# sec-bit/ckb-zkp

Measured on AMD Instinct MI355X. Metric: Groth16 proofs/sec (2^20 constraints, BN256), higher is better.
Workload: dtype u32 limbs (256-bit Montgomery integers); 1 GPU; Groth16 prove, MiMC-chain R1CS, 1048570 constraints (domain 2^20), 1258284 aux, bn254, G1 x4 + G2 x1 MSM + 4 NTT (7 in the reference: evaluation-form key); curve=bn254, log_domain=20, parallelism=independent proofs x1

## Files before the change

### ckb_zkp_amd/csrc/capi.hip

```cpp
#include <cstdint>
#include <cstdlib>
#include <cstring>

#include "ctx.hpp"
#include "host_field.hpp"
#include "internal.hpp"
#include "ipa.hpp"

using namespace zkp;

namespace {

template <class Fn>
int32_t guarded(zkp_ctx* ctx, Fn&& fn) {
  if (!ctx) return ZKP_ERR_BAD_ARG;
  std::lock_guard<std::recursive_mutex> lk(ctx->mu);
  try {
    ZKP_HIP(hipSetDevice(ctx->device));
    fn();
    return ZKP_OK;
  } catch (const StatusError& e) {
    return e.status;
  } catch (const HipError& e) {
    ctx->last_error = std::string(e.what) + ": " + hipGetErrorString(e.e);
    fprintf(stderr, "[zkp_accel] HIP error %s at line %d: %s\n", hipGetErrorString(e.e), e.line, e.what);
    return e.e == hipErrorOutOfMemory ? ZKP_ERR_OOM : ZKP_ERR_DEVICE;
  } catch (const std::bad_alloc&) {
    return ZKP_ERR_OOM;
  } catch (...) {
    return ZKP_ERR_DEVICE;
  }
}

template <class Fn>
int32_t guarded_multi(zkp_ctx* root, Fn&& fn) {
  if (!root) return ZKP_ERR_BAD_ARG;
  std::vector<std::unique_lock<std::recursive_mutex>> member_locks;
  std::unique_lock<std::recursive_mutex> root_lock(root->mu);
  for (size_t k = 1; k < root->devs.size(); k++) member_locks.emplace_back(root->devs[k]->mu);
  return guarded(root, fn);
}

zkp_cfg cfg_from_env() {
  zkp_cfg c;
  auto num = [](const char* name, long long dflt) { const char* e = getenv(name); return e ? atoll(e) : dflt; };
  auto off = [](const char* name) { const char* e = getenv(name); return e && atoi(e) == 0; };
  c.lanes = (int)num("ZKP_LANES", 0);
  c.msm_batch_lanes = (int)std::max<long long>(1, std::min<long long>(num("ZKP_BATCH_LANES", 1), zkp_ctx::N_LANES));
  c.msm_c = (int)num("ZKP_MSM_C", 0);
  c.msm_c_g2 = (int)num("ZKP_MSM_C_G2", 0);
  if (const char* e = getenv("ZKP_MSM_CHUNK")) c.msm_chunk = (long long)strtoull(e, nullptr, 0);
  if (const char* e = getenv("ZKP_TABLE_BUDGET_GB")) c.table_budget_gb = atof(e);
  c.h_lagrange = !off("ZKP_H_LAGRANGE");
  c.c_fold = !off("ZKP_C_FOLD");
  c.host_affine = !off("ZKP_HOST_AFFINE");
  c.lfold_heavy_cost = num("ZKP_LFOLD_HEAVY_COST", c.lfold_heavy_cost);
  if (const char* e = getenv("ZKP_MULTI_EXCHANGE")) c.multi_exchange = !strcmp(e, "rccl") ? ZKP_EXCHANGE_RCCL : !strcmp(e, "peer") ? ZKP_EXCHANGE_PEER : ZKP_EXCHANGE_AUTO;
  c.multi_exchange_timeout_ms = (int)num("ZKP_MULTI_EXCHANGE_TIMEOUT_MS", c.multi_exchange_timeout_ms);
  c.multi_wm_split = (int)num("ZKP_MULTI_WM_SPLIT", -1);
  return c;
}

int32_t apply_config(zkp_cfg* c, const zkp_ctx_config* u) {
  if (!u) return ZKP_OK;
  if (u->struct_size < sizeof(uint32_t) * 2) return ZKP_ERR_BAD_ARG;
  zkp_ctx_config f{};
  memcpy(&f, u, std::min<size_t>(u->struct_size, sizeof f));
  auto tri_ok = [](int32_t v) { return v == ZKP_DEFAULT || v == ZKP_ON || v == ZKP_OFF; };
  if (f.lanes < 0 || f.lanes > zkp_ctx::N_LANES || f.msm_batch_lanes < 0 || f.msm_batch_lanes > zkp_ctx::N_LANES) return ZKP_ERR_BAD_ARG;
  for (int32_t b : {f.msm_window_bits, f.msm_window_bits_g2})
    if (b != 0 && (b < 2 || b > 22)) return ZKP_ERR_BAD_ARG;
  if (f.msm_chunk_points < -1 || (f.msm_chunk_points > 0 && f.msm_chunk_points < 1024)) return ZKP_ERR_BAD_ARG;
  if (!(f.table_budget_gb >= 0.0) || f.c_fold_heavy_cost < 0 || f.multi_exchange_timeout_ms < 0) return ZKP_ERR_BAD_ARG;
  if (!tri_ok(f.h_evaluation_form) || !tri_ok(f.c_fold) || !tri_ok(f.host_affine) || !tri_ok(f.multi_witness_split)) return ZKP_ERR_BAD_ARG;
  if (f.multi_exchange < ZKP_EXCHANGE_AUTO || f.multi_exchange > ZKP_EXCHANGE_PEER) return ZKP_ERR_BAD_ARG;
  if (f.lanes) c->lanes = f.lanes;
  if (f.msm_batch_lanes) c->msm_batch_lanes = f.msm_batch_lanes;
  if (f.msm_window_bits) c->msm_c = f.msm_window_bits;
  if (f.msm_window_bits_g2) c->msm_c_g2 = f.msm_window_bits_g2;
  if (f.msm_chunk_points) c->msm_chunk = f.msm_chunk_points < 0 ? 0 : f.msm_chunk_points;
  if (f.table_budget_gb > 0.0) c->table_budget_gb = f.table_budget_gb;
  if (f.h_evaluation_form) c->h_lagrange = f.h_evaluation_form == ZKP_ON;
  if (f.c_fold) c->c_fold = f.c_fold == ZKP_ON;
  if (f.host_affine) c->host_affine = f.host_affine == ZKP_ON;
  if (f.c_fold_heavy_cost) c->lfold_heavy_cost = f.c_fold_heavy_cost;
  if (f.multi_exchange) c->multi_exchange = f.multi_exchange;
  if (f.multi_exchange_timeout_ms) c->multi_exchange_timeout_ms = f.multi_exchange_timeout_ms;
  if (f.multi_witness_split) c->multi_wm_split = f.multi_witness_split == ZKP_ON ? 1 : 0;
  return ZKP_OK;
}

}

extern "C" {

const char* zkp_status_string(int32_t s) {
  switch (s) {
    case ZKP_OK: return "ok";
    case ZKP_ERR_BAD_ARG: return "bad argument";
    case ZKP_ERR_UNSUPPORTED_CURVE: return "unsupported curve";
    case ZKP_ERR_DOMAIN_TOO_LARGE: return "domain too large (PolynomialDegreeTooLarge)";
    case ZKP_ERR_OOM: return "out of device memory";
    case ZKP_ERR_DEVICE: return "HIP device error / no gfx950 device (there is no CPU fallback)";
    case ZKP_ERR_BAD_HANDLE: return "bad handle";
    case ZKP_ERR_INVALID_POINT: return "malformed point / not on the curve / not in the prime-order subgroup (InvalidData)";
    default: return "unknown status";
  }
}

const char* zkp_version(void) { return "zkp_accel 0.7.1 (gfx950)"; }

int32_t zkp_ctx_get_config(zkp_ctx* ctx, zkp_ctx_config* out) {
  if (!ctx || !out) return ZKP_ERR_BAD_ARG;
  return guarded(ctx, [&] {
    const zkp_cfg& c = ctx->cfg;
    zkp_ctx_config f{};
    f.struct_size = sizeof f;
    f.lanes = c.lanes;
    f.msm_batch_lanes = c.msm_batch_lanes;
    f.msm_window_bits = c.msm_c;
    f.msm_window_bits_g2 = c.msm_c_g2;
    f.msm_chunk_points = c.msm_chunk > 0 ? c.msm_chunk : -1;
    f.table_budget_gb = c.table_budget_gb;
    f.h_evaluation_form = c.h_lagrange ? ZKP_ON : ZKP_OFF;
    f.c_fold = c.c_fold ? ZKP_ON : ZKP_OFF;
    f.host_affine = c.host_affine ? ZKP_ON : ZKP_OFF;
    f.c_fold_heavy_cost = c.lfold_heavy_cost;
    f.multi_exchange = c.multi_exchange;
    f.multi_exchange_timeout_ms = c.multi_exchange_timeout_ms;
    f.multi_witness_split = c.multi_wm_split < 0 ? ZKP_DEFAULT : c.multi_wm_split ? ZKP_ON : ZKP_OFF;
    *out = f;
  });
}

int32_t zkp_ctx_create(zkp_ctx** out, int device_id) { return zkp_ctx_create_ex(out, device_id, nullptr); }

int32_t zkp_ctx_create_ex(zkp_ctx** out, int device_id, const zkp_ctx_config* user_cfg) {
  if (!out) return ZKP_ERR_BAD_ARG;
  *out = nullptr;
  zkp_cfg cfg = cfg_from_env();
  if (int32_t st = apply_config(&cfg, user_cfg); st != ZKP_OK) return st;
  int count = 0;
  if (hipGetDeviceCount(&count) != hipSuccess || count <= 0 || device_id < 0 || device_id >= count) {
    fprintf(stderr, "[zkp_accel] no usable HIP device (count=%d, requested %d); there is no CPU fallback\n", count,
            device_id);
    return ZKP_ERR_DEVICE;
  }
  zkp_ctx* ctx = new (std::nothrow) zkp_ctx();
  if (!ctx) return ZKP_ERR_OOM;
  ctx->device = device_id;
  ctx->cfg = cfg;
  int32_t st = guarded(ctx, [&] {
    ZKP_HIP(hipEventCreate(&ctx->ev0));
    ZKP_HIP(hipEventCreate(&ctx->ev1));
    ZKP_HIP(hipEventCreate(&ctx->ev2));
    ZKP_HIP(hipEventCreate(&ctx->ev3));
    for (int l = 0; l < zkp_ctx::N_LANES; l++) {
      zkp_lane& L = ctx->lanes[l];
      ZKP_HIP(hipStreamCreateWithFlags(&L.stream, hipStreamNonBlocking));
      ZKP_HIP(hipEventCreateWithFlags(&L.ev_fork, hipEventDisableTiming));
      ZKP_HIP(hipEventCreateWithFlags(&L.ev_a, hipEventDisableTiming));
      ZKP_HIP(hipEventCreateWithFlags(&L.ev_b1, hipEventDisableTiming));
      ZKP_HIP(hipHostMalloc(reinterpret_cast<void**>(&L.host_proof), 1100));
      for (int i = 0; i < zkp_lane::N_WS; i++) {
        ZKP_HIP(hipEventCreateWithFlags(&L.ws[i].done, hipEventDisableTiming));
        ZKP_HIP(hipEventCreateWithFlags(&L.ws[i].sorted, hipEventDisableTiming));
        ZKP_HIP(hipEventCreateWithFlags(&L.ws[i].l1_done, hipEventDisableTiming));
        ZKP_HIP(hipEventCreateWithFlags(&L.ws[i].acc_done, hipEventDisableTiming));
        if (i > 0) {
          ZKP_HIP(hipStreamCreateWithFlags(&L.ws[i].stream, hipStreamNonBlocking));
          L.ws[i].own_stream = true;
        }
      }
    }
  });
  if (st != ZKP_OK) {
    (void)zkp_ctx_destroy(ctx);
    return st;
  }
  *out = ctx;
  return ZKP_OK;
}

int32_t zkp_ctx_create_multi(zkp_ctx** out, const int* device_ids, int n_devices) {
  return zkp_ctx_create_multi_ex(out, device_ids, n_devices, nullptr);
}

int32_t zkp_ctx_create_multi_ex(zkp_ctx** out, const int* device_ids, int n_devices, const zkp_ctx_config* cfg) {
  if (!out || !device_ids || n_devices < 1 || n_devices > 64) return ZKP_ERR_BAD_ARG;
  *out = nullptr;
  zkp_ctx* root = nullptr;
  int32_t st = zkp_ctx_create_ex(&root, device_ids[0], cfg);
  if (st != ZKP_OK) return st;
  root->devs.push_back(root);
  for (int k = 1; k < n_devices; k++) {
    zkp_ctx* m = nullptr;
    st = zkp_ctx_create_ex(&m, device_ids[k], cfg);
    if (st != ZKP_OK) {
      (void)zkp_ctx_destroy(root);
      return st;
    }
    root->devs.push_back(m);
  }
  for (int a = 0; a < n_devices; a++)
    for (int b = 0; b < n_devices; b++) {
      if (device_ids[a] == device_ids[b]) continue;
      int can = 0;
      if (hipDeviceCanAccessPeer(&can, device_ids[a], device_ids[b]) == hipSuccess && can) {
        (void)hipSetDevice(device_ids[a]);
        hipError_t e = hipDeviceEnablePeerAccess(device_ids[b], 0);
        if (e != hipSuccess) (void)hipGetLastError();
      }
    }
  (void)hipSetDevice(device_ids[0]);
  *out = root;
  return ZKP_OK;
}
int32_t zkp_ctx_num_devices(zkp_ctx* ctx, int32_t* n) {
  if (!ctx || !n) return ZKP_ERR_BAD_ARG;
  *n = ctx->devs.empty() ? 1 : (int32_t)ctx->devs.size();
  return ZKP_OK;
}
int32_t zkp_ctx_device(zkp_ctx* ctx, int32_t rank, zkp_ctx** member) {
  if (!ctx || !member) return ZKP_ERR_BAD_ARG;
  if (ctx->devs.empty()) {
    if (rank != 0) return ZKP_ERR_BAD_ARG;
    *member = ctx;
    return ZKP_OK;
  }
  if (rank < 0 || rank >= (int32_t)ctx->devs.size()) return ZKP_ERR_BAD_ARG;
  *member = ctx->devs[rank];
  return ZKP_OK;
}

int32_t zkp_ctx_destroy(zkp_ctx* ctx) {
  if (!ctx) return ZKP_ERR_BAD_ARG;
  { std::lock_guard<std::recursive_mutex> wait_for_calls_in_flight(ctx->mu); }
  for (size_t k = 1; k < ctx->devs.size(); k++) (void)zkp_ctx_destroy(ctx->devs[k]);
  ctx->devs.clear();
  (void)hipSetDevice(ctx->device);
  (void)hipDeviceSynchronize();
  ntt_free_tables(ctx);
  msm_free_all(ctx);
  for (hipEvent_t e : {ctx->ev0, ctx->ev1, ctx->ev2, ctx->ev3})
    if (e) (void)hipEventDestroy(e);
  for (int l = 0; l < zkp_ctx::N_LANES; l++) {
    zkp_lane& L = ctx->lanes[l];
    for (hipEvent_t e : {L.ev_fork, L.ev_a, L.ev_b1})
      if (e) (void)hipEventDestroy(e);
    if (L.host_proof) (void)hipHostFree(L.host_proof);
    for (int i = 0; i < zkp_lane::N_WS; i++) {
      if (L.ws[i].done) (void)hipEventDestroy(L.ws[i].done);
      if (L.ws[i].sorted) (void)hipEventDestroy(L.ws[i].sorted);
      if (L.ws[i].l1_done) (void)hipEventDestroy(L.ws[i].l1_done);
      if (L.ws[i].acc_done) (void)hipEventDestroy(L.ws[i].acc_done);
      if (L.ws[i].own_stream && L.ws[i].stream) (void)hipStreamDestroy(L.ws[i].stream);
    }
    if (L.own_stream && L.stream) (void)hipStreamDestroy(L.stream);
  }
  if (ctx->pinned) (void)hipHostFree(ctx->pinned);
  delete ctx;
  return ZKP_OK;
}

int32_t zkp_ctx_set_stream(zkp_ctx* ctx, void* s) {
  return guarded(ctx, [&] {
    zkp_lane& L = ctx->lanes[0];
    ZKP_HIP(hipStreamSynchronize(L.stream));
    if (s) {
      if (L.own_stream && L.stream) (void)hipStreamDestroy(L.stream);
      L.stream = reinterpret_cast<hipStream_t>(s);
      L.own_stream = false;
    } else if (!L.own_stream) {
      ZKP_HIP(hipStreamCreateWithFlags(&L.stream, hipStreamNonBlocking));
      L.own_stream = true;
    }
  });
}

int32_t zkp_ctx_sync(zkp_ctx* ctx) {
  return guarded(ctx, [&] { ZKP_HIP(hipStreamSynchronize(ctx->cur->stream)); });
}

int32_t zkp_dev_alloc(zkp_ctx* ctx, size_t bytes, void** dptr) {
  if (!dptr) return ZKP_ERR_BAD_ARG;
  return guarded(ctx, [&] {
    *dptr = nullptr;
    if (hipMalloc(dptr, bytes ? bytes : 16) != hipSuccess) throw StatusError{ZKP_ERR_OOM};
  });
}
int32_t zkp_dev_free(zkp_ctx* ctx, void* dptr) {
  return guarded(ctx, [&] {
    ZKP_HIP(hipStreamSynchronize(ctx->cur->stream));
    if (dptr) ZKP_HIP(hipFree(dptr));
  });
}
int32_t zkp_h2d(zkp_ctx* ctx, void* dst, const void* src, size_t bytes) {
  if (bytes && (!dst || !src)) return ZKP_ERR_BAD_ARG;
  return guarded(ctx, [&] {
    if (bytes) ZKP_HIP(hipMemcpyAsync(dst, src, bytes, hipMemcpyHostToDevice, ctx->cur->stream));
    ZKP_HIP(hipStreamSynchronize(ctx->cur->stream));
  });
}
int32_t zkp_d2h(zkp_ctx* ctx, void* dst, const void* src, size_t bytes) {
  if (bytes && (!dst || !src)) return ZKP_ERR_BAD_ARG;
  return guarded(ctx, [&] {
    if (bytes) ZKP_HIP(hipMemcpyAsync(dst, src, bytes, hipMemcpyDeviceToHost, ctx->cur->stream));
    ZKP_HIP(hipStreamSynchronize(ctx->cur->stream));
  });
}
int32_t zkp_timer_start(zkp_ctx* ctx) {
  return guarded(ctx, [&] { ZKP_HIP(hipEventRecord(ctx->ev0, ctx->cur->stream)); });
// ... 423 lines not shown
```

### ckb_zkp_amd/csrc/ctx.hpp

```cpp
#pragma once
#include <hip/hip_runtime.h>
#include <stdint.h>

#include <map>
#include <mutex>
#include <memory>
#include <string>
#include <unordered_map>
#include <vector>

#include "../../include/zkp_accel.h"

namespace zkp {

struct HipError {
  hipError_t e;
  const char* what;
  int line;
};

#define ZKP_HIP(call)                                                   \
  do {                                                                  \
    hipError_t _e = (call);                                             \
    if (_e != hipSuccess) throw ::zkp::HipError{_e, #call, __LINE__};   \
// ... 32 lines not shown
  DevBuf& operator=(const DevBuf&) = delete;
};

struct NttTables {
  int log_n = 0, h = 0;
  uint32_t* w_lo = nullptr;
  uint32_t* w_hi = nullptr;
  uint32_t* wi_lo = nullptr;
  uint32_t* wi_hi = nullptr;
  uint32_t* g_lo = nullptr;
  uint32_t* g_hi = nullptr;
  uint32_t* gi_lo = nullptr;
  uint32_t* gi_hi = nullptr;
  uint32_t* sub_fwd = nullptr;
  uint32_t* sub_inv = nullptr;
  uint32_t* n_inv = nullptr;
  void* block = nullptr;
  uint32_t* full_fwd[8] = {};
  uint32_t* full_inv[8] = {};
  uint32_t* full_g = nullptr;
  uint32_t* full_gi = nullptr;
  uint32_t* g_hi_n = nullptr;
  uint32_t* full_g_n = nullptr;
  std::vector<void*> extra;
};

struct BasesEntry;

struct MsmWorkspace {
  hipStream_t stream = nullptr;
  bool own_stream = false;
  hipEvent_t done = nullptr;
  hipEvent_t sorted = nullptr;
  hipEvent_t l1_done = nullptr;
  uint32_t chain_nb = 0;
  size_t chain_xb = 0;
  hipEvent_t acc_done = nullptr;
  DevBuf keys, vals, keys2, vals2, sort_tmp, offsets, buckets, tmp, out, sched, scan_tmp, scan_tmp2, partial, redo;
};
struct Groth16Timing {
  zkp_groth16_timing t{};
};

}

struct zkp_lane {
  hipStream_t stream = nullptr;
  bool own_stream = true;
  static constexpr int N_WS = 4;
  static constexpr int N_WS_MSM = N_WS;
  zkp::MsmWorkspace ws[N_WS];
  zkp::DevBuf ntt_scratch;
  hipEvent_t ev_fork = nullptr, ev_a = nullptr, ev_b1 = nullptr;
  uint32_t* host_proof = nullptr;
  bool host_tail = false;
  bool busy = false;
};

struct zkp_cfg {
  int lanes = 0;
  int msm_batch_lanes = 1;
  int msm_c = 0, msm_c_g2 = 0;
  long long msm_chunk = (long long)3 << 19;
  double table_budget_gb = 0;
  bool h_lagrange = true, c_fold = true, host_affine = true;
  long long lfold_heavy_cost = 0;
  int multi_exchange = 0;
  int multi_exchange_timeout_ms = 30000;
  int multi_wm_split = -1;
};

struct zkp_ctx {
  int device = 0;
  zkp_cfg cfg;
  std::recursive_mutex mu;
  static constexpr int N_LANES = 8;
  static constexpr int N_WS = zkp_lane::N_WS;
  zkp_lane lanes[N_LANES];
  zkp_lane* cur = &lanes[0];
  int cur_idx = 0;
  hipEvent_t ev0 = nullptr, ev1 = nullptr;
  hipEvent_t ev2 = nullptr, ev3 = nullptr;
  bool profiling = false;
  size_t table_bytes = 0;
  bool msm_defer_reduce = false;
  int msm_acc_into = -1;
  int msm_bucket_ws = -1;
  bool dbg_skip_k8 = false;
  bool batch_mode = false;
  std::map<std::pair<int, int>, zkp::NttTables> ntt_tables;
  zkp::DevBuf ntt_io, poly_tmp, poly_consts, spmv_list;
  zkp::DevBuf msm_scalars, msm_misc, var_bases;
  uint32_t* pinned = nullptr;
  size_t pinned_cap = 0;
  std::unordered_map<uint64_t, std::shared_ptr<zkp::BasesEntry>> bases;
  uint64_t next_handle = 1;
  zkp_groth16_timing last_timing{};
  zkp_marlin_timing last_marlin_timing{};
  std::string last_error;
  std::vector<zkp_ctx*> devs;
  std::map<std::pair<int, int>, std::shared_ptr<void>> var_plans;
  bool tl_on = false;
  std::string tl_tag;
  std::vector<std::pair<std::string, hipEvent_t>> tl;
  void mark(hipStream_t st, const char* what) {
    if (!tl_on) return;
    hipEvent_t e = nullptr;
    if (hipEventCreate(&e) != hipSuccess) return;
    (void)hipEventRecord(e, st);
    tl.emplace_back(tl_tag + what, e);
  }
};
```

### ckb_zkp_amd/csrc/groth16.hip

```cpp
#include <algorithm>
#include <cstdlib>
#include <cstring>
#include <memory>
#include <string>
#include <vector>

#include "field_dev.hpp"
#include "host_field.hpp"
#include "internal.hpp"
#include "msm_vtbl.hpp"

using namespace zkp;

struct DevCsr {
  uint32_t* row_ptr = nullptr;
  uint32_t* col = nullptr;
  uint32_t* coeff = nullptr;
  size_t nnz = 0;
};

struct zkp_groth16_pk {
  int curve = 0;
  uint32_t num_inputs = 0, num_aux = 0, num_constraints = 0;
  int log_n = 0;
// ... 606 lines not shown
    return hq;
  }
  hipLaunchKernelGGL(qap_pointwise_kernel<P>, dim3((N + 255) / 256), dim3(256), 0, st, a, b, c,
                     pk->consts.as<uint32_t>(64), N);
  ntt_run(ctx, pk->curve, a, pk->log_n, ZKP_NTT_COSET_IFFT);
  ZKP_HIP(hipGetLastError());
  return a;
}

void groth16_witness_map(zkp_ctx* ctx, zkp_groth16_pk* pk, const uint64_t* z, uint64_t* h, bool on_device) {
  const uint32_t* zd = reinterpret_cast<const uint32_t*>(z);
  if (!on_device) {
    uint32_t* s = pk->lane[ctx->cur_idx].S.as<uint32_t>((pk->nz + 4) * 8);
    ZKP_HIP(hipMemcpyAsync(s, z, pk->nz * 32, hipMemcpyHostToDevice, ctx->cur->stream));
    zd = s;
  }
  uint32_t* hd = pk->curve == ZKP_BN254 ? witness_map_dev<Bn254Fr>(ctx, pk, zd) : witness_map_dev<Bls381Fr>(ctx, pk, zd);
  ZKP_HIP(hipMemcpyAsync(h, hd, pk->N * 32, on_device ? hipMemcpyDeviceToDevice : hipMemcpyDeviceToHost, ctx->cur->stream));
  if (!on_device) ZKP_HIP(hipStreamSynchronize(ctx->cur->stream));
}

template <class FrP>
static void prove_enqueue_part(zkp_ctx* ctx, zkp_groth16_pk* pk, const uint64_t* z, bool z_on_device, const uint64_t* r,
                               const uint64_t* s, int part, char* partial_out = nullptr, bool latency_plan = false) {
  ZKP_REQUIRE((pk->shard_world > 0) == (partial_out != nullptr), ZKP_ERR_BAD_ARG);
  ZKP_REQUIRE(pk->hA != 0, ZKP_ERR_BAD_ARG);
  zkp_groth16_pk::PerLane& PL = pk->lane[ctx->cur_idx];
  hipStream_t st = ctx->cur->stream;
  const bool prof = ctx->profiling;
  const bool host_tail = ctx->cfg.host_affine && !partial_out;
  zkp_groth16_timing tm{};
  struct ProfEvents {
    hipEvent_t e[4] = {nullptr, nullptr, nullptr, nullptr};
    ~ProfEvents() {
      for (hipEvent_t x : e)
        if (x) (void)hipEventDestroy(x);
    }
  } pev;
  if (prof)
    for (hipEvent_t& x : pev.e) ZKP_HIP(hipEventCreate(&x));
  hipEvent_t &e0 = pev.e[0], &e1 = pev.e[1], &eT0 = pev.e[2], &eT1 = pev.e[3];
  auto tic = [&] { if (prof) ZKP_HIP(hipEventRecord(e0, st)); };
  auto toc = [&](float* dst) {
    if (!prof) return;
    ZKP_HIP(hipEventRecord(e1, st));
    ZKP_HIP(hipEventSynchronize(e1));
    ZKP_HIP(hipEventElapsedTime(dst, e0, e1));
  };
  if (prof) ZKP_HIP(hipEventRecord(eT0, st));
  uint32_t* S = PL.S.as<uint32_t>((pk->nz + 4) * 8);
  uint32_t* rs = PL.proof.as<uint32_t>(1024);
  uint32_t* proof_dev = rs + 16;
  uint32_t* flags_dev = proof_dev + 256;
  if (part & 1) {
    ZKP_HIP(hipMemcpyAsync(S, z, pk->nz * 32, z_on_device ? hipMemcpyDeviceToDevice : hipMemcpyHostToDevice, st));
    ZKP_HIP(hipMemcpyAsync(rs, r, 32, hipMemcpyHostToDevice, st));
    ZKP_HIP(hipMemcpyAsync(rs + 8, s, 32, hipMemcpyHostToDevice, st));
  }
  if (!(part & 2)) return;
  hipLaunchKernelGGL(scalar_tail_kernel<FrP>, dim3(1), dim3(64), 0, st, S + pk->nz * 8, rs);

  const MsmVtbl* v1 = msm_vtbl(pk->curve, 1);
  const MsmVtbl* v2 = msm_vtbl(pk->curve, 2);
  const size_t slot = v2->xyzz_bytes;
  char* res = reinterpret_cast<char*>(PL.results.get(6 * slot));
  const uint64_t* Sd = reinterpret_cast<const uint64_t*>(S);
  bool l_done_in_fan = false, g2_done_in_fan = false, chained = false;
  float acc_ms = 0.f, scan_ms = 0.f;
  uint64_t ent = 0, scan_bytes = 0, scan_runs = 0;
  static const bool single_stream = getenv("ZKP_SINGLE_STREAM") && atoi(getenv("ZKP_SINGLE_STREAM")) != 0;
  const bool fan = !prof && !single_stream;
  uint32_t* h = nullptr;
  auto run = [&](int idx, uint64_t handle, const uint64_t* sc, size_t n, int w, int sort_src = -1, int l1_src = -1) {
    float ms = 0.f, ms_sc = 0.f;
    uint64_t e = 0;
    static const char* const names[5] = {"A", "B1", "B2", "H", "L"};
    ctx->tl_tag = names[idx];
    tic();
#ifdef ZKP_ABLATION
    static const int skip_k8 = [] { const char* e = getenv("ZKP_DEBUG_SKIP_K8_MASK"); return e ? (int)strtol(e, nullptr, 0) : 0; }();
    ctx->dbg_skip_k8 = ((skip_k8 >> idx) & 1) && ctx->batch_mode;
#endif
    msm_run(ctx, handle, 0, sc, n, true, nullptr, res + idx * slot, prof ? &ms : nullptr, &e, fan ? w : 0,
            fan ? sort_src : -1, prof ? &ms_sc : nullptr, fan ? l1_src : -1);
    ctx->dbg_skip_k8 = false;
    toc(&tm.ms_msm[idx]);
    acc_ms += ms;
    ent += e;
    tm.ms_msm_acc[idx] = ms;
    tm.msm_entries[idx] = e;
    if (ms_sc > 0.f) {
      scan_ms += ms_sc;
      scan_bytes += 2 * 32 * (uint64_t)n + 8 * e;
      scan_runs += 1;
    }
    tm.msm_accumulate_launches += 1;
  };
  ctx->tl_tag.clear();
  ctx->mark(st, "start");
  if (fan) {
    ZKP_HIP(hipEventRecord(ctx->cur->ev_fork, st));
    for (int w = 1; w < zkp_ctx::N_WS; w++) ZKP_HIP(hipStreamWaitEvent(ctx->cur->ws[w].stream, ctx->cur->ev_fork, 0));
    static const bool wm_first = !(getenv("ZKP_WM_FIRST") && atoi(getenv("ZKP_WM_FIRST")) == 0);
    if (wm_first) {
      h = witness_map_dev<FrP>(ctx, pk, S, !pk->h_lagrange);
      ctx->mark(st, "wm");
    }
    static const bool l_own = !(getenv("ZKP_L_OWN_STREAM") && atoi(getenv("ZKP_L_OWN_STREAM")) == 0);
    static const int lat_env = [] { const char* e = getenv("ZKP_LATENCY_PLAN"); return e ? atoi(e) : -1; }();
    (void)latency_plan;
    const bool lat = lat_env >= 0 ? lat_env != 0 : true;
    if (lat) {
      const int l1 = pk->share_l1 ? 1 : -1;
      const bool b_l1 = pk->share_l1 && pk->b_in_l1;
      if (!b_l1) run(2, pk->hB2, Sd + 4 * pk->q_lo[2], pk->q_n[2], 2);
      run(0, pk->hA, Sd + 4 * pk->q_lo[0], pk->q_n[0], 1);
      ZKP_HIP(hipEventRecord(ctx->cur->ev_a, ctx->cur->ws[1].stream));
      if (b_l1) run(2, pk->hB2, Sd + 4 * pk->q_lo[2], pk->q_n[2], 2, -1, l1);
      static const bool g2_early = !(getenv("ZKP_G2_EARLY") && atoi(getenv("ZKP_G2_EARLY")) == 0);
      if (!partial_out && g2_early && !host_tail) {
        v2->assemble_g2(ctx->cur->ws[2].stream, res, slot, proof_dev, flags_dev, 2 * v1->fN);
        g2_done_in_fan = true;
      }
      run(1, pk->hB1, Sd + 4 * pk->q_lo[1], pk->q_n[1], 3, pk->share_b_sort ? 2 : -1);
      ctx->msm_defer_reduce = chained = pk->chain_lh;
      run(4, pk->hL, Sd + 4 * pk->q_lo[4], pk->q_n[4], 1, pk->share_al_sort ? 1 : -1, l1);
      if (!partial_out) {
        ZKP_HIP(hipStreamWaitEvent(ctx->cur->ws[3].stream, ctx->cur->ev_a, 0));
        v1->assemble_g1_part1(ctx->cur->ws[3].stream, res, slot, rs, host_tail ? nullptr : proof_dev, flags_dev);
        ctx->tl_tag.clear();
        ctx->mark(ctx->cur->ws[3].stream, "part1");
      }
    } else {
    run(2, pk->hB2, Sd + 4 * pk->q_lo[2], pk->q_n[2], 2);
    run(0, pk->hA, Sd + 4 * pk->q_lo[0], pk->q_n[0], 1);
    run(1, pk->hB1, Sd + 4 * pk->q_lo[1], pk->q_n[1], 1, pk->share_b_sort ? 2 : -1);
    if (l_own) run(4, pk->hL, Sd + 4 * pk->q_lo[4], pk->q_n[4], 3, pk->share_al_sort && pk->share_b_sort ? 1 : -1);
    ZKP_HIP(hipEventRecord(ctx->cur->ev_b1, ctx->cur->ws[1].stream));
    if (!partial_out) {
      ZKP_HIP(hipStreamWaitEvent(ctx->cur->ws[3].stream, ctx->cur->ev_b1, 0));
      v1->assemble_g1_part1(ctx->cur->ws[3].stream, res, slot, rs, host_tail ? nullptr : proof_dev, flags_dev);
    }
    }
    l_done_in_fan = lat || l_own;
  }
  tic();
  if (!h) h = witness_map_dev<FrP>(ctx, pk, S, !pk->h_lagrange);
  toc(&tm.ms_witness_map);
  if (!fan) {
    run(0, pk->hA, Sd + 4 * pk->q_lo[0], pk->q_n[0], 0);
    run(1, pk->hB1, Sd + 4 * pk->q_lo[1], pk->q_n[1], 0);
    run(2, pk->hB2, Sd + 4 * pk->q_lo[2], pk->q_n[2], 0);
  }
  if (chained) ctx->msm_acc_into = 1;
  run(3, pk->hH, reinterpret_cast<const uint64_t*>(h) + 4 * pk->q_lo[3], pk->q_n[3], 0);
  if (!(fan && l_done_in_fan)) run(4, pk->hL, Sd + 4 * pk->q_lo[4], pk->q_n[4], 0);
  if (fan) {
    for (int w = 1; w < zkp_ctx::N_WS; w++) {
      ZKP_HIP(hipEventRecord(ctx->cur->ws[w].done, ctx->cur->ws[w].stream));
      ZKP_HIP(hipStreamWaitEvent(st, ctx->cur->ws[w].done, 0));
    }
  }
  tm.ms_msm_accumulate = acc_ms;
  tm.msm_points = ent;
  tm.ms_msm_scan = scan_ms;
  tm.msm_scan_bytes = scan_bytes;
  tm.msm_scan_launches = scan_runs;
  if (partial_out) {
    ZKP_HIP(hipMemcpyAsync(partial_out, res, 5 * slot, hipMemcpyDeviceToDevice, st));
    ZKP_HIP(hipGetLastError());
    if (prof) {
      ZKP_HIP(hipEventRecord(eT1, st));
      ZKP_HIP(hipStreamSynchronize(st));
      ZKP_HIP(hipEventElapsedTime(&tm.ms_total, eT0, eT1));
      ctx->last_timing = tm;
    }
    return;
  }

  tic();
  if (!fan) v1->assemble_g1_part1(st, res, slot, rs, host_tail ? nullptr : proof_dev, flags_dev);
  v1->assemble_g1_part2(st, res, slot, host_tail ? nullptr : proof_dev, flags_dev, 2 * v1->fN + 2 * v2->fN);
  if (!g2_done_in_fan && !host_tail) v2->assemble_g2(st, res, slot, proof_dev, flags_dev, 2 * v1->fN);
  ZKP_HIP(hipGetLastError());
  toc(&tm.ms_assemble);
  const size_t proof_words = 4 * (size_t)v1->fN + 2 * (size_t)v2->fN;
  if (host_tail) {
    uint32_t* hp = ctx->cur->host_proof;
    ZKP_HIP(hipMemcpyAsync(hp, res, 16 * (size_t)v1->fN, hipMemcpyDeviceToHost, st));
    ZKP_HIP(hipMemcpyAsync(hp + 4 * v1->fN, res + 2 * slot, 16 * (size_t)v2->fN, hipMemcpyDeviceToHost, st));
    ZKP_HIP(hipMemcpyAsync(hp + 4 * v1->fN + 4 * v2->fN, res + 5 * slot, 16 * (size_t)v1->fN, hipMemcpyDeviceToHost, st));
  } else {
    ZKP_HIP(hipMemcpyAsync(ctx->cur->host_proof, proof_dev, proof_words * 4, hipMemcpyDeviceToHost, st));
    ZKP_HIP(hipMemcpyAsync(ctx->cur->host_proof + 256, flags_dev, 12, hipMemcpyDeviceToHost, st));
  }
  ctx->tl_tag.clear();
  ctx->mark(st, "copied");
  ctx->cur->host_tail = host_tail;
  ctx->cur->busy = true;
  if (prof) {
    ZKP_HIP(hipEventRecord(eT1, st));
    ZKP_HIP(hipStreamSynchronize(st));
    ZKP_HIP(hipEventElapsedTime(&tm.ms_total, eT0, eT1));
    ctx->last_timing = tm;
  }
}

static std::vector<const void*> lane_signature(zkp_ctx* ctx, zkp_groth16_pk* pk) {
  std::vector<const void*> sig;
  zkp_lane* L = ctx->cur;
  zkp_groth16_pk::PerLane& PL = pk->lane[ctx->cur_idx];
  for (DevBuf* b : {&PL.abc, &PL.S, &PL.results, &PL.proof, &L->ntt_scratch}) sig.push_back(b->p);
  for (int w = 0; w < zkp_lane::N_WS; w++) {
    MsmWorkspace& ws = L->ws[w];
    for (DevBuf* b : {&ws.keys, &ws.vals, &ws.keys2, &ws.vals2, &ws.sort_tmp, &ws.offsets, &ws.buckets, &ws.tmp, &ws.out,
                      &ws.sched, &ws.scan_tmp, &ws.scan_tmp2, &ws.partial, &ws.redo})
      sig.push_back(b->p);
  }
  sig.push_back(pk);
  return sig;
}

template <class FrP>
static void prove_enqueue(zkp_ctx* ctx, zkp_groth16_pk* pk, const uint64_t* z, bool z_on_device, const uint64_t* r,
                          const uint64_t* s, bool latency_plan = false) {
  static const bool graph_on = getenv("ZKP_GRAPH") && atoi(getenv("ZKP_GRAPH")) != 0;
  static const bool single_stream = getenv("ZKP_SINGLE_STREAM") && atoi(getenv("ZKP_SINGLE_STREAM")) != 0;
  if (!graph_on || ctx->profiling || single_stream) {
    prove_enqueue_part<FrP>(ctx, pk, z, z_on_device, r, s, 3, nullptr, latency_plan);
    return;
  }
  zkp_groth16_pk::PerLane& PL = pk->lane[ctx->cur_idx];
  hipStream_t st = ctx->cur->stream;
  if (PL.graph_state == 2 && PL.sig == lane_signature(ctx, pk)) {
    prove_enqueue_part<FrP>(ctx, pk, z, z_on_device, r, s, 1);
    ZKP_HIP(hipGraphLaunch(PL.graph_exec, st));
    ctx->cur->busy = true;
    return;
  }
  if (PL.graph_state == 2) {
    (void)hipGraphExecDestroy(PL.graph_exec);
    (void)hipGraphDestroy(PL.graph);
    PL.graph_exec = nullptr;
    PL.graph = nullptr;
    PL.graph_state = 0;
  }
  if (PL.graph_state == 1 && PL.sig == lane_signature(ctx, pk)) {
    prove_enqueue_part<FrP>(ctx, pk, z, z_on_device, r, s, 1);
    ZKP_HIP(hipStreamBeginCapture(st, hipStreamCaptureModeRelaxed));
    try {
      prove_enqueue_part<FrP>(ctx, pk, z, z_on_device, r, s, 2);
    } catch (...) {
      hipGraph_t g = nullptr;
      (void)hipStreamEndCapture(st, &g);
      if (g) (void)hipGraphDestroy(g);
      throw;
    }
    ZKP_HIP(hipStreamEndCapture(st, &PL.graph));
    ZKP_HIP(hipGraphInstantiate(&PL.graph_exec, PL.graph, nullptr, nullptr, 0));
    PL.graph_state = 2;
    ZKP_HIP(hipGraphLaunch(PL.graph_exec, st));
    ctx->cur->busy = true;
    return;
  }
  prove_enqueue_part<FrP>(ctx, pk, z, z_on_device, r, s, 3);
  PL.sig = lane_signature(ctx, pk);
  PL.graph_state = 1;
}

static void prove_finish(zkp_ctx* ctx, zkp_groth16_pk* pk, uint64_t* proof_out, uint8_t* inf_out) {
  const MsmVtbl* v1 = msm_vtbl(pk->curve, 1);
  const MsmVtbl* v2 = msm_vtbl(pk->curve, 2);
  const size_t proof_words = 4 * (size_t)v1->fN + 2 * (size_t)v2->fN;
  ZKP_HIP(hipStreamSynchronize(ctx->cur->stream));
  if (!ctx->tl.empty()) {
    std::string line = "[zkp timeline ms]";
    for (auto& m : ctx->tl) {
      float ms = 0.f;
      (void)hipEventSynchronize(m.second);
      (void)hipEventElapsedTime(&ms, ctx->tl[0].second, m.second);
      char buf[64];
      snprintf(buf, sizeof buf, " %s=%.2f", m.first.c_str(), ms);
      line += buf;
      if (&m != &ctx->tl[0]) (void)hipEventDestroy(m.second);
    }
    (void)hipEventDestroy(ctx->tl[0].second);
    ctx->tl.clear();
    fprintf(stderr, "%s\n", line.c_str());
  }
  if (ctx->cur->host_tail) {
    const hostf::HostField Fq = hostf::fq_field(pk->curve);
    const uint32_t* hp = ctx->cur->host_proof;
    hostf::groth16_points_into_affine(Fq, hp, hp + 4 * v1->fN, hp + 4 * v1->fN + 4 * v2->fN,
                                      reinterpret_cast<uint32_t*>(proof_out), inf_out);
  } else {
    memcpy(proof_out, ctx->cur->host_proof, proof_words * 4);
    for (int i = 0; i < 3; i++) inf_out[i] = (uint8_t)ctx->cur->host_proof[256 + i];
  }
  ctx->cur->busy = false;
}

void groth16_assemble(zkp_ctx* ctx, int curve, const uint64_t* sums, const uint64_t* r, const uint64_t* s,
                      uint64_t* proof_out, uint8_t* inf_out) {
  const MsmVtbl* v1 = msm_vtbl(curve, 1);
  const MsmVtbl* v2 = msm_vtbl(curve, 2);
  hipStream_t st = ctx->cur->stream;
  const size_t slot = v2->xyzz_bytes;
  const size_t j1 = 3 * (size_t)v1->fN, j2 = 3 * (size_t)v2->fN;
  const size_t in_words = 4 * j1 + j2;
  uint32_t* buf = ctx->msm_misc.as<uint32_t>(in_words + 16 + 6 * slot / 4 + 256 + 16);
  uint32_t* jac = buf;
  uint32_t* rs = jac + in_words;
  char* res = reinterpret_cast<char*>(rs + 16);
  uint32_t* proof_dev = reinterpret_cast<uint32_t*>(res + 6 * slot);
  uint32_t* flags_dev = proof_dev + 240;
  ZKP_HIP(hipMemcpyAsync(jac, sums, in_words * 4, hipMemcpyHostToDevice, st));
  ZKP_HIP(hipMemcpyAsync(rs, r, 32, hipMemcpyHostToDevice, st));
  ZKP_HIP(hipMemcpyAsync(rs + 8, s, 32, hipMemcpyHostToDevice, st));
  const size_t off[5] = {0, j1, 2 * j1, 2 * j1 + j2, 3 * j1 + j2};
  for (int i = 0; i < 5; i++) (i == 2 ? v2 : v1)->from_jacobian(st, jac + off[i], res + i * slot);
  v1->assemble_g1_part1(st, res, slot, rs, proof_dev, flags_dev);
  v1->assemble_g1_part2(st, res, slot, proof_dev, flags_dev, 2 * v1->fN + 2 * v2->fN);
  v2->assemble_g2(st, res, slot, proof_dev, flags_dev, 2 * v1->fN);
  ZKP_HIP(hipGetLastError());
  const size_t proof_words = 4 * (size_t)v1->fN + 2 * (size_t)v2->fN;
  uint32_t flags_host[4] = {0, 0, 0, 0};
  ZKP_HIP(hipMemcpyAsync(proof_out, proof_dev, proof_words * 4, hipMemcpyDeviceToHost, st));
// ... 5 lines not shown
size_t groth16_partials_bytes(int curve) { return 5 * msm_vtbl(curve, 2)->xyzz_bytes; }

void groth16_prove_partials(zkp_ctx* ctx, zkp_groth16_pk* pk, const uint64_t* z_dev, const uint64_t* r, const uint64_t* s,
                            void* out_dev) {
  ZKP_REQUIRE(pk->shard_world > 0, ZKP_ERR_BAD_ARG);
  ctx->cur = &ctx->lanes[0];
  ctx->cur_idx = 0;
  if (pk->curve == ZKP_BN254) prove_enqueue_part<Bn254Fr>(ctx, pk, z_dev, true, r, s, 3, (char*)out_dev, true);
  else prove_enqueue_part<Bls381Fr>(ctx, pk, z_dev, true, r, s, 3, (char*)out_dev, true);
  ZKP_HIP(hipStreamSynchronize(ctx->cur->stream));
}

void groth16_fold_assemble(zkp_ctx* ctx, int curve, const void* gathered_dev, int world, const uint64_t* r,
                           const uint64_t* s, uint64_t* proof_out, uint8_t* inf_out) {
  ZKP_REQUIRE(world >= 1, ZKP_ERR_BAD_ARG);
  const MsmVtbl* v1 = msm_vtbl(curve, 1);
  const MsmVtbl* v2 = msm_vtbl(curve, 2);
  hipStream_t st = ctx->cur->stream;
  const size_t slot = v2->xyzz_bytes;
  uint32_t* buf = ctx->msm_misc.as<uint32_t>(16 + 6 * slot / 4 + 256 + 16);
  uint32_t* rs = buf;
  char* res = reinterpret_cast<char*>(rs + 16);
  uint32_t* proof_dev = reinterpret_cast<uint32_t*>(res + 6 * slot);
  uint32_t* flags_dev = proof_dev + 240;
  ZKP_HIP(hipMemcpyAsync(rs, r, 32, hipMemcpyHostToDevice, st));
  ZKP_HIP(hipMemcpyAsync(rs + 8, s, 32, hipMemcpyHostToDevice, st));
  v1->fold_slots(st, (const char*)gathered_dev, 5 * slot, world, slot, 0x1b, res);
  v2->fold_slots(st, (const char*)gathered_dev, 5 * slot, world, slot, 0x04, res);
  v1->assemble_g1_part1(st, res, slot, rs, proof_dev, flags_dev);
  v1->assemble_g1_part2(st, res, slot, proof_dev, flags_dev, 2 * v1->fN + 2 * v2->fN);
  v2->assemble_g2(st, res, slot, proof_dev, flags_dev, 2 * v1->fN);
  ZKP_HIP(hipGetLastError());
  const size_t proof_words = 4 * (size_t)v1->fN + 2 * (size_t)v2->fN;
  uint32_t flags_host[4] = {0, 0, 0, 0};
  ZKP_HIP(hipMemcpyAsync(proof_out, proof_dev, proof_words * 4, hipMemcpyDeviceToHost, st));
  ZKP_HIP(hipMemcpyAsync(flags_host, flags_dev, 12, hipMemcpyDeviceToHost, st));
  ZKP_HIP(hipStreamSynchronize(st));
  for (int i = 0; i < 3; i++) inf_out[i] = (uint8_t)flags_host[i];
}

void groth16_prove(zkp_ctx* ctx, zkp_groth16_pk* pk, const uint64_t* z, bool z_on_device, const uint64_t* r,
                   const uint64_t* s, uint64_t* proof_out, uint8_t* inf_out) {
  ZKP_REQUIRE(pk->shard_world == 0, ZKP_ERR_BAD_ARG);
  ctx->cur = &ctx->lanes[0];
  ctx->cur_idx = 0;
  static const bool timeline = getenv("ZKP_TIMELINE") && atoi(getenv("ZKP_TIMELINE")) != 0;
  ctx->tl_on = timeline && !ctx->profiling;
  if (pk->curve == ZKP_BN254) prove_enqueue<Bn254Fr>(ctx, pk, z, z_on_device, r, s, true);
  else prove_enqueue<Bls381Fr>(ctx, pk, z, z_on_device, r, s, true);
  ctx->tl_on = false;
  prove_finish(ctx, pk, proof_out, inf_out);
}

void groth16_prove_batch(zkp_ctx* ctx, zkp_groth16_pk* pk, size_t n, const uint64_t* const* z_dev, const uint64_t* r,
                         const uint64_t* s, uint64_t* proofs_out, uint8_t* inf_out, bool z_on_device) {
  const MsmVtbl* v1 = msm_vtbl(pk->curve, 1);
  const MsmVtbl* v2 = msm_vtbl(pk->curve, 2);
  const size_t pw64 = (4 * (size_t)v1->fN + 2 * (size_t)v2->fN) / 2;
  const bool prof = ctx->profiling;
  ZKP_REQUIRE(pk->shard_world == 0, ZKP_ERR_BAD_ARG);
  size_t pending[zkp_ctx::N_LANES] = {};
  const int lanes_default = pk->log_n <= 22 ? 8 : 4;
  const int nl = std::max(1, std::min(ctx->cfg.lanes > 0 ? ctx->cfg.lanes : lanes_default, (int)zkp_ctx::N_LANES));
  auto select = [&](int l) {
    ctx->cur = &ctx->lanes[l];
    ctx->cur_idx = l;
  };
  struct BatchMode {
    zkp_ctx* c;
    ~BatchMode() { c->batch_mode = false; }
  } batch_mode{ctx};
  ctx->batch_mode = n > 1 && !prof;
  try {
    if (ctx->batch_mode) {
      std::vector<uint64_t> scratch_proof(pw64 + 8);
      uint8_t scratch_inf[4];
      bool any = false;
      for (int l = 0; l < nl; l++) {
        if (pk->lane[l].warmed) continue;
        select(l);
        if (pk->curve == ZKP_BN254) prove_enqueue<Bn254Fr>(ctx, pk, z_dev[0], z_on_device, r, s);
        else prove_enqueue<Bls381Fr>(ctx, pk, z_dev[0], z_on_device, r, s);
        pk->lane[l].warmed = true;
        any = true;
      }
      if (any)
        for (int l = 0; l < nl; l++) {
          select(l);
          if (ctx->cur->busy) prove_finish(ctx, pk, scratch_proof.data(), scratch_inf);
        }
    }
    for (size_t i = 0; i < n; i++) {
      const int l = prof ? 0 : (int)(i % nl);
      select(l);
      if (ctx->cur->busy) prove_finish(ctx, pk, proofs_out + pending[l] * pw64, inf_out + pending[l] * 3);
      if (pk->curve == ZKP_BN254) prove_enqueue<Bn254Fr>(ctx, pk, z_dev[i], z_on_device, r + 4 * i, s + 4 * i);
      else prove_enqueue<Bls381Fr>(ctx, pk, z_dev[i], z_on_device, r + 4 * i, s + 4 * i);
      pending[l] = i;
    }
    for (int l = 0; l < zkp_ctx::N_LANES; l++) {
      select(l);
      if (ctx->cur->busy) prove_finish(ctx, pk, proofs_out + pending[l] * pw64, inf_out + pending[l] * 3);
    }
  } catch (...) {
    (void)hipDeviceSynchronize();
    for (auto& L : ctx->lanes) L.busy = false;
    select(0);
    throw;
  }
  select(0);
}

}
#include <dlfcn.h>

#include <chrono>
#include <condition_variable>
#include <mutex>
#include <string>

#include <thread>
struct zkp_groth16_pk_multi {
  int mode = 0, curve = 0;
  std::vector<zkp_groth16_pk*> pk;
  std::vector<hipEvent_t> ev_chain, ev_done, ev_h_read;
// ... 482 lines not shown
```

Baseline: 142.8 proofs/s.

## Map batch lanes onto a fixed set of role streams when hardware queues are few

```diff
diff --git a/ckb_zkp_amd/csrc/capi.hip b/ckb_zkp_amd/csrc/capi.hip
--- a/ckb_zkp_amd/csrc/capi.hip
+++ b/ckb_zkp_amd/csrc/capi.hip
@@ -58,6 +58,14 @@
   if (const char* e = getenv("ZKP_MULTI_EXCHANGE")) c.multi_exchange = !strcmp(e, "rccl") ? ZKP_EXCHANGE_RCCL : !strcmp(e, "peer") ? ZKP_EXCHANGE_PEER : ZKP_EXCHANGE_AUTO;
   c.multi_exchange_timeout_ms = (int)num("ZKP_MULTI_EXCHANGE_TIMEOUT_MS", c.multi_exchange_timeout_ms);
   c.multi_wm_split = (int)num("ZKP_MULTI_WM_SPLIT", -1);
+  const long long q = num("GPU_MAX_HW_QUEUES", 4);
+  c.hw_queues = q >= 1 ? (int)std::min<long long>(q, 1 << 20) : 4;
+  c.role_plan = c.hw_queues < 16;
+  if (const char* e = getenv("ZKP_STREAM_PLAN")) {
+    if (!strcmp(e, "roles")) c.role_plan = true;
+    else if (!strcmp(e, "lanes")) c.role_plan = false;
+  }
+  c.role_opt = (int)num("ZKP_ROLE_OPT", 0);
   return c;
 }
 
@@ -155,13 +163,16 @@
     ZKP_HIP(hipEventCreate(&ctx->ev1));
     ZKP_HIP(hipEventCreate(&ctx->ev2));
     ZKP_HIP(hipEventCreate(&ctx->ev3));
+    if (ctx->cfg.role_plan)
+      for (hipStream_t& r : ctx->role) ZKP_HIP(hipStreamCreateWithFlags(&r, hipStreamNonBlocking));
     for (int l = 0; l < zkp_ctx::N_LANES; l++) {
       zkp_lane& L = ctx->lanes[l];
       ZKP_HIP(hipStreamCreateWithFlags(&L.stream, hipStreamNonBlocking));
+      ZKP_HIP(hipEventCreateWithFlags(&L.ev_done, hipEventDisableTiming));
       ZKP_HIP(hipEventCreateWithFlags(&L.ev_fork, hipEventDisableTiming));
       ZKP_HIP(hipEventCreateWithFlags(&L.ev_a, hipEventDisableTiming));
       ZKP_HIP(hipEventCreateWithFlags(&L.ev_b1, hipEventDisableTiming));
-      ZKP_HIP(hipHostMalloc(reinterpret_cast<void**>(&L.host_proof), 1100));
+      ZKP_HIP(hipHostMalloc(reinterpret_cast<void**>(&L.host_proof), zkp_lane::HOST_PROOF_BYTES));
       for (int i = 0; i < zkp_lane::N_WS; i++) {
         ZKP_HIP(hipEventCreateWithFlags(&L.ws[i].done, hipEventDisableTiming));
         ZKP_HIP(hipEventCreateWithFlags(&L.ws[i].sorted, hipEventDisableTiming));
@@ -246,7 +257,7 @@
     if (e) (void)hipEventDestroy(e);
   for (int l = 0; l < zkp_ctx::N_LANES; l++) {
     zkp_lane& L = ctx->lanes[l];
-    for (hipEvent_t e : {L.ev_fork, L.ev_a, L.ev_b1})
+    for (hipEvent_t e : {L.ev_fork, L.ev_a, L.ev_b1, L.ev_done})
       if (e) (void)hipEventDestroy(e);
     if (L.host_proof) (void)hipHostFree(L.host_proof);
     for (int i = 0; i < zkp_lane::N_WS; i++) {
@@ -258,6 +269,8 @@
     }
     if (L.own_stream && L.stream) (void)hipStreamDestroy(L.stream);
   }
+  for (hipStream_t r : ctx->role)
+    if (r) (void)hipStreamDestroy(r);
   if (ctx->pinned) (void)hipHostFree(ctx->pinned);
   delete ctx;
   return ZKP_OK;
diff --git a/ckb_zkp_amd/csrc/ctx.hpp b/ckb_zkp_amd/csrc/ctx.hpp
--- a/ckb_zkp_amd/csrc/ctx.hpp
+++ b/ckb_zkp_amd/csrc/ctx.hpp
@@ -108,7 +108,12 @@
   zkp::MsmWorkspace ws[N_WS];
   zkp::DevBuf ntt_scratch;
   hipEvent_t ev_fork = nullptr, ev_a = nullptr, ev_b1 = nullptr;
+  hipEvent_t ev_done = nullptr;
+  bool wait_ev_done = false;
+  hipStream_t in_stream = nullptr;
   uint32_t* host_proof = nullptr;
+  static constexpr int HOST_RS = 264;
+  static constexpr size_t HOST_PROOF_BYTES = (HOST_RS + 16) * 4;
   bool host_tail = false;
   bool busy = false;
 };
@@ -124,6 +129,9 @@
   int multi_exchange = 0;
   int multi_exchange_timeout_ms = 30000;
   int multi_wm_split = -1;
+  int hw_queues = 4;
+  bool role_plan = true;
+  int role_opt = 0;
 };
 
 struct zkp_ctx {
@@ -135,6 +143,10 @@
   zkp_lane lanes[N_LANES];
   zkp_lane* cur = &lanes[0];
   int cur_idx = 0;
+  static constexpr int N_ROLES = 4;
+  enum { ROLE_FILL0 = 0, ROLE_FILL1 = 1, ROLE_G2 = 2, ROLE_TAIL = 3 };
+  hipStream_t role[N_ROLES] = {};
+  bool roles_on = false;
   hipEvent_t ev0 = nullptr, ev1 = nullptr;
   hipEvent_t ev2 = nullptr, ev3 = nullptr;
   bool profiling = false;
diff --git a/ckb_zkp_amd/csrc/groth16.hip b/ckb_zkp_amd/csrc/groth16.hip
--- a/ckb_zkp_amd/csrc/groth16.hip
+++ b/ckb_zkp_amd/csrc/groth16.hip
@@ -682,13 +682,30 @@
   uint32_t* rs = PL.proof.as<uint32_t>(1024);
   uint32_t* proof_dev = rs + 16;
   uint32_t* flags_dev = proof_dev + 256;
-  if (part & 1) {
+  const bool roles = ctx->roles_on;
+  ZKP_REQUIRE(!roles || (part == 3 && !prof && !partial_out), ZKP_ERR_BAD_ARG);
+  const int ropt = roles ? ctx->cfg.role_opt : 0;
+  hipStream_t sin = roles && (ropt & 2) ? ctx->cur->ws[1].stream : st;
+  hipStream_t tail = roles ? ctx->role[zkp_ctx::ROLE_TAIL] : st;
+  if (roles) {
+    uint32_t* hrs = ctx->cur->host_proof + zkp_lane::HOST_RS;
+    memcpy(hrs, r, 32);
+    memcpy(hrs + 8, s, 32);
+    if (!z_on_device) {
+      ZKP_HIP(hipMemcpyAsync(S, z, pk->nz * 32, hipMemcpyHostToDevice, ctx->cur->in_stream));
+      ZKP_HIP(hipEventRecord(ctx->cur->ev_fork, ctx->cur->in_stream));
+      ZKP_HIP(hipStreamWaitEvent(sin, ctx->cur->ev_fork, 0));
+    } else {
+      ZKP_HIP(hipMemcpyAsync(S, z, pk->nz * 32, hipMemcpyDeviceToDevice, sin));
+    }
+    ZKP_HIP(hipMemcpyAsync(rs, hrs, 64, hipMemcpyHostToDevice, sin));
+  } else if (part & 1) {
     ZKP_HIP(hipMemcpyAsync(S, z, pk->nz * 32, z_on_device ? hipMemcpyDeviceToDevice : hipMemcpyHostToDevice, st));
     ZKP_HIP(hipMemcpyAsync(rs, r, 32, hipMemcpyHostToDevice, st));
     ZKP_HIP(hipMemcpyAsync(rs + 8, s, 32, hipMemcpyHostToDevice, st));
   }
   if (!(part & 2)) return;
-  hipLaunchKernelGGL(scalar_tail_kernel<FrP>, dim3(1), dim3(64), 0, st, S + pk->nz * 8, rs);
+  hipLaunchKernelGGL(scalar_tail_kernel<FrP>, dim3(1), dim3(64), 0, sin, S + pk->nz * 8, rs);
 
   const MsmVtbl* v1 = msm_vtbl(pk->curve, 1);
   const MsmVtbl* v2 = msm_vtbl(pk->curve, 2);
@@ -729,8 +746,10 @@
   ctx->tl_tag.clear();
   ctx->mark(st, "start");
   if (fan) {
-    ZKP_HIP(hipEventRecord(ctx->cur->ev_fork, st));
-    for (int w = 1; w < zkp_ctx::N_WS; w++) ZKP_HIP(hipStreamWaitEvent(ctx->cur->ws[w].stream, ctx->cur->ev_fork, 0));
+    ZKP_HIP(hipEventRecord(ctx->cur->ev_fork, sin));
+    if (sin != st) ZKP_HIP(hipStreamWaitEvent(st, ctx->cur->ev_fork, 0));
+    for (int w = 1; w < zkp_ctx::N_WS; w++)
+      if (ctx->cur->ws[w].stream != sin) ZKP_HIP(hipStreamWaitEvent(ctx->cur->ws[w].stream, ctx->cur->ev_fork, 0));
     static const bool wm_first = !(getenv("ZKP_WM_FIRST") && atoi(getenv("ZKP_WM_FIRST")) == 0);
     if (wm_first) {
       h = witness_map_dev<FrP>(ctx, pk, S, !pk->h_lagrange);
@@ -739,7 +758,7 @@
     static const bool l_own = !(getenv("ZKP_L_OWN_STREAM") && atoi(getenv("ZKP_L_OWN_STREAM")) == 0);
     static const int lat_env = [] { const char* e = getenv("ZKP_LATENCY_PLAN"); return e ? atoi(e) : -1; }();
     (void)latency_plan;
-    const bool lat = lat_env >= 0 ? lat_env != 0 : true;
+    const bool lat = roles || (lat_env >= 0 ? lat_env != 0 : true);
     if (lat) {
       const int l1 = pk->share_l1 ? 1 : -1;
       const bool b_l1 = pk->share_l1 && pk->b_in_l1;
@@ -752,14 +771,21 @@
         v2->assemble_g2(ctx->cur->ws[2].stream, res, slot, proof_dev, flags_dev, 2 * v1->fN);
         g2_done_in_fan = true;
       }
-      run(1, pk->hB1, Sd + 4 * pk->q_lo[1], pk->q_n[1], 3, pk->share_b_sort ? 2 : -1);
+      auto run_b1 = [&] { run(1, pk->hB1, Sd + 4 * pk->q_lo[1], pk->q_n[1], 3, pk->share_b_sort && !(ropt & 4) ? 2 : -1); };
+      if (!roles) run_b1();
       ctx->msm_defer_reduce = chained = pk->chain_lh;
       run(4, pk->hL, Sd + 4 * pk->q_lo[4], pk->q_n[4], 1, pk->share_al_sort ? 1 : -1, l1);
+      if (roles) {
+        run_b1();
+        ZKP_HIP(hipEventRecord(ctx->cur->ev_b1, ctx->cur->ws[3].stream));
+        ZKP_HIP(hipStreamWaitEvent(tail, ctx->cur->ev_b1, 0));
+      }
       if (!partial_out) {
-        ZKP_HIP(hipStreamWaitEvent(ctx->cur->ws[3].stream, ctx->cur->ev_a, 0));
-        v1->assemble_g1_part1(ctx->cur->ws[3].stream, res, slot, rs, host_tail ? nullptr : proof_dev, flags_dev);
+        hipStream_t p1 = roles ? tail : ctx->cur->ws[3].stream;
+        ZKP_HIP(hipStreamWaitEvent(p1, ctx->cur->ev_a, 0));
+        v1->assemble_g1_part1(p1, res, slot, rs, host_tail ? nullptr : proof_dev, flags_dev);
         ctx->tl_tag.clear();
-        ctx->mark(ctx->cur->ws[3].stream, "part1");
+        ctx->mark(p1, "part1");
       }
     } else {
     run(2, pk->hB2, Sd + 4 * pk->q_lo[2], pk->q_n[2], 2);
@@ -786,11 +812,13 @@
   run(3, pk->hH, reinterpret_cast<const uint64_t*>(h) + 4 * pk->q_lo[3], pk->q_n[3], 0);
   if (!(fan && l_done_in_fan)) run(4, pk->hL, Sd + 4 * pk->q_lo[4], pk->q_n[4], 0);
   if (fan) {
-    for (int w = 1; w < zkp_ctx::N_WS; w++) {
-      ZKP_HIP(hipEventRecord(ctx->cur->ws[w].done, ctx->cur->ws[w].stream));
-      ZKP_HIP(hipStreamWaitEvent(st, ctx->cur->ws[w].done, 0));
-    }
-  }
+    for (int w = roles ? 0 : 1; w < zkp_ctx::N_WS; w++) {
+      hipStream_t sw = w == 0 ? st : ctx->cur->ws[w].stream;
+      ZKP_HIP(hipEventRecord(ctx->cur->ws[w].done, sw));
+      ZKP_HIP(hipStreamWaitEvent(tail, ctx->cur->ws[w].done, 0));
+    }
+  }
+  if (roles) st = tail;
   tm.ms_msm_accumulate = acc_ms;
   tm.msm_points = ent;
   tm.ms_msm_scan = scan_ms;
@@ -828,6 +856,8 @@
   ctx->mark(st, "copied");
   ctx->cur->host_tail = host_tail;
   ctx->cur->busy = true;
+  ctx->cur->wait_ev_done = roles;
+  if (roles) ZKP_HIP(hipEventRecord(ctx->cur->ev_done, st));
   if (prof) {
     ZKP_HIP(hipEventRecord(eT1, st));
     ZKP_HIP(hipStreamSynchronize(st));
@@ -902,7 +932,9 @@
   const MsmVtbl* v1 = msm_vtbl(pk->curve, 1);
   const MsmVtbl* v2 = msm_vtbl(pk->curve, 2);
   const size_t proof_words = 4 * (size_t)v1->fN + 2 * (size_t)v2->fN;
-  ZKP_HIP(hipStreamSynchronize(ctx->cur->stream));
+  if (ctx->cur->wait_ev_done) ZKP_HIP(hipEventSynchronize(ctx->cur->ev_done));
+  else ZKP_HIP(hipStreamSynchronize(ctx->cur->stream));
+  ctx->cur->wait_ev_done = false;
   if (!ctx->tl.empty()) {
     std::string line = "[zkp timeline ms]";
     for (auto& m : ctx->tl) {
@@ -1014,6 +1046,7 @@
   prove_finish(ctx, pk, proof_out, inf_out);
 }
 
+static constexpr int ROLE_LANES_DEFAULT = 4;
 void groth16_prove_batch(zkp_ctx* ctx, zkp_groth16_pk* pk, size_t n, const uint64_t* const* z_dev, const uint64_t* r,
                          const uint64_t* s, uint64_t* proofs_out, uint8_t* inf_out, bool z_on_device) {
   const MsmVtbl* v1 = msm_vtbl(pk->curve, 1);
@@ -1022,8 +1055,15 @@
   const bool prof = ctx->profiling;
   ZKP_REQUIRE(pk->shard_world == 0, ZKP_ERR_BAD_ARG);
   size_t pending[zkp_ctx::N_LANES] = {};
-  const int lanes_default = pk->log_n <= 22 ? 8 : 4;
+  static const bool graph_on = getenv("ZKP_GRAPH") && atoi(getenv("ZKP_GRAPH")) != 0;
+  static const bool single_stream = getenv("ZKP_SINGLE_STREAM") && atoi(getenv("ZKP_SINGLE_STREAM")) != 0;
+  const bool use_roles = ctx->cfg.role_plan && ctx->role[0] && !prof && !graph_on && !single_stream;
+  const int lanes_default = use_roles ? ROLE_LANES_DEFAULT : pk->log_n <= 22 ? 8 : 4;
   const int nl = std::max(1, std::min(ctx->cfg.lanes > 0 ? ctx->cfg.lanes : lanes_default, (int)zkp_ctx::N_LANES));
+  static const bool dbg_plan = getenv("ZKP_DEBUG_PLAN") && atoi(getenv("ZKP_DEBUG_PLAN")) != 0;
+  if (dbg_plan)
+    fprintf(stderr, "[zkp_accel] prove_batch: plan=%s lanes=%d hw_queues=%d log_n=%d\n", use_roles ? "roles" : "lanes", nl,
+            ctx->cfg.hw_queues, pk->log_n);
   auto select = [&](int l) {
     ctx->cur = &ctx->lanes[l];
     ctx->cur_idx = l;
@@ -1033,6 +1073,42 @@
     ~BatchMode() { c->batch_mode = false; }
   } batch_mode{ctx};
   ctx->batch_mode = n > 1 && !prof;
+  struct RolePlan {
+    zkp_ctx* c;
+    bool on = false;
+    hipStream_t saved[zkp_ctx::N_LANES][zkp_lane::N_WS] = {};
+    explicit RolePlan(zkp_ctx* ctx) : c(ctx) {}
+    void enter() {
+      const bool b1_on_g2 = (c->cfg.role_opt & 1) != 0;
+      for (int l = 0; l < zkp_ctx::N_LANES; l++) {
+        zkp_lane& L = c->lanes[l];
+        saved[l][0] = L.stream;
+        for (int w = 1; w < zkp_lane::N_WS; w++) saved[l][w] = L.ws[w].stream;
+        L.in_stream = L.stream;
+        L.stream = c->role[zkp_ctx::ROLE_FILL0];
+        L.ws[1].stream = c->role[zkp_ctx::ROLE_FILL1];
+        L.ws[2].stream = c->role[zkp_ctx::ROLE_G2];
+        L.ws[3].stream = c->role[b1_on_g2 ? zkp_ctx::ROLE_G2 : zkp_ctx::ROLE_FILL1];
+      }
+      on = c->roles_on = true;
+    }
+    ~RolePlan() {
+      if (!on) return;
+      for (int l = 0; l < zkp_ctx::N_LANES; l++) {
+        zkp_lane& L = c->lanes[l];
+        L.stream = saved[l][0];
+        for (int w = 1; w < zkp_lane::N_WS; w++) L.ws[w].stream = saved[l][w];
+        L.in_stream = nullptr;
+        L.wait_ev_done = false;
+      }
+      c->roles_on = false;
+    }
+  } role_plan{ctx};
+  if (use_roles) {
+    ZKP_HIP(hipEventRecord(ctx->lanes[0].ev_done, ctx->lanes[0].stream));
+    for (hipStream_t r : ctx->role) ZKP_HIP(hipStreamWaitEvent(r, ctx->lanes[0].ev_done, 0));
+    role_plan.enter();
+  }
   try {
     if (ctx->batch_mode) {
       std::vector<uint64_t> scratch_proof(pw64 + 8);
```

New measurement: 142.7 proofs/s. Within noise of the previous version (-0.1%).
